# THGLab/NewtonNet

Hardware: AMD Instinct MI355X
Metric: atom-steps/sec (energy+force) on batched MD17 aspirin (higher is better)
Workload: dtype f32; 1 GPU; MD17 aspirin batched inference, 1024 conformers x 21 atoms per GPU, fp32, energy+force, neighbor list included (BASELINE.json configs[1]); 2 independent step(s) in flight per GPU; atoms_per_gpu=21504, weights=seed0, distinct_batches=4, steps_in_flight=2, parallelism=1 independent shard(s), no data-path collective

## Files before the change

newtonnet_amd/csrc/common.h:

```cpp
#pragma once
#include <hip/hip_runtime.h>
#include <stdint.h>

#include "../../include/newtonnet_hip.h"

#if (defined(EDGE_ABL_SELF) || defined(EDGE_ABL_PAIR) || defined(EDGE_ABL_TABLE) || defined(EDGE_ABL_STORE) ||              \
     defined(EDGE_ABL_NO_TABLE) || defined(EDGE_ABL_HALF_TABLE) || defined(EDGE_ABL_NOTAB) || defined(EDGE_ABL_NOMJ) || defined(MLPS_ABL_NO_H) || defined(NS_ABL_NO_Q) || defined(NS_ABL_HOT_W) || defined(MLPS_ABL_X) || defined(ABL_NO_SILU) || defined(ABL_NO_STORE) ||                  \
     (defined(LIN_ABLATE_NO_LOAD) && LIN_ABLATE_NO_LOAD) || (defined(LIN_ABLATE_NO_STORE) && LIN_ABLATE_NO_STORE) ||         \
     (defined(LIN_ABLATE_NO_MFMA) && LIN_ABLATE_NO_MFMA) || (defined(LIN_ABLATE_NO_LDS) && LIN_ABLATE_NO_LDS)) &&            \
    !defined(NNHIP_TOOLING)
#error "ablation switches produce wrong results: build through csrc/build.sh (it marks the library with -DNNHIP_TOOLING)"
#endif

#define NF NNHIP_F
#define NB NNHIP_NB
#define WAVE 64
#ifndef FT_G
#define FT_G 3072
#endif
#define FT_ROWS (FT_G + 8)
#define FT_ZERO_ROW (FT_G + 3)
#define FT_PLANE ((size_t)FT_ROWS * NNHIP_F)

typedef float f32x16 __attribute__((ext_vector_type(16)));
// ... 296 lines not shown
#define WIMG_FMT_SPLIT_F16 0
#define WIMG_FMT_BF16 1
#define WIMG_MAX_JOBS 40
struct WeightImageJobs {
  const float* src[WIMG_MAX_JOBS];
  char* dst[WIMG_MAX_JOBS];
  int fmt;
};
enum { IMG_UPDATE = 0, IMG_NODE0, IMG_NODE2, IMG_UPDATE_T, IMG_NODE0_T, IMG_NODE2_T, IMG_EQ1_0, IMG_EQ1_2, IMG_EQ2_0, IMG_EQ2_2,
       IMG_EQ1_0_T, IMG_EQ1_2_T, IMG_EQ2_0_T, IMG_EQ2_2_T, IMG_PER_LAYER };
enum { IMG_HEAD0 = 0, IMG_HEAD2, IMG_HEAD0_T, IMG_HEAD2_T, IMG_HEAD_COUNT };
struct NodeImages {
  const char *Wu, *W0, *W2;
  const char *W2T, *W0T, *WuT;
};
int launch_weight_images(const float* const* src, char* const* dst, int n, hipStream_t s, int fmt = WIMG_FMT_SPLIT_F16);
int launch_node_fwd_split(const NodeFwdArgs& a, const NodeImages& im, hipStream_t s);
int launch_node_bwd_split(const NodeBwdArgs& a, const NodeImages& im, hipStream_t s);
struct NodeTurnArgs {
  const float* f;
  const float* a_mid;
  float* a_out;
  const float *b0, *b2;
  const float *w4, *b4;
  const float *scale, *shift;
  const int64_t* z;
  float* atom_energy;
  float* g_a;
  float* gf;
  int N;
};
int launch_node_turn_split(const NodeTurnArgs& a, const NodeImages& im, hipStream_t s);
bool node_turn_enabled();
int launch_mlp_wide_split(int mode, bool accum, const MlpArgs& a, hipStream_t s);
int launch_mlp_wide_pair_split(int mode, const MlpPair& P, hipStream_t s);
int launch_lin_wide_split(const float* X, int ldx, const char* img, float* Y, int ldy, int M, bool acc, hipStream_t s);
bool split_products_enabled();

struct MsgBwdForceTail {
  const float* g_u;
  const float* geo;
  const int* rev;
  int n_edges, n_layers;
  float inv_rc;
  float* forces;
};

static inline int cdiv(long a, long b) { return (int)((a + b - 1) / b); }
```

newtonnet_amd/csrc/node128.hip:

```cpp
#include <string.h>

#include "common.h"

#ifndef NODE_WG_PER_CU
#define NODE_WG_PER_CU 2
#endif
#define NT_LD 132
#define NODE_LDS_FLOATS (32 * NT_LD)

struct Tile {
  float* xs;
  int r, h, nb;
};

__device__ __forceinline__ void load_w(float4 (&wf)[16], const Tile& t, const float* __restrict__ W) {
  const float4* wp = reinterpret_cast<const float4*>(W + (size_t)(t.nb * 32 + t.r) * NF + 4 * t.h);
#pragma unroll
  for (int k = 0; k < 16; ++k) wf[k] = wp[2 * k];
  __builtin_amdgcn_sched_barrier(0);
}

__device__ __forceinline__ f32x16 tile_gemm(const Tile& t, const float4 (&wf)[16]) {
  f32x16 acc;
#pragma unroll
// ... 57 lines not shown

__global__ void __launch_bounds__(256, NODE_WG_PER_CU) node_fwd_kernel(const NodeFwdArgs p) {
  __shared__ __attribute__((aligned(16))) float xs[NODE_LDS_FLOATS];
  Tile t;
  t.xs = xs;
  t.r = threadIdx.x & 31;
  t.h = (threadIdx.x >> 5) & 1;
  t.nb = __builtin_amdgcn_readfirstlane(threadIdx.x >> 6);
  const int row = blockIdx.x * 32 + t.r;
  const int rc = min(row, p.N - 1);
  const bool live = row < p.N;

  float4 wf[16];
  load_w(wf, t, p.Wu);
  float upd[16];
#pragma unroll
  for (int k = 0; k < 16; ++k) upd[k] = 0.f;
  float xa[16], xb[16], a[16];
  blk_load(xa, p.f, ((size_t)rc * 3 + 0) * NF, t);
#pragma unroll
  for (int c = 0; c < 3; ++c) {
    float (&cur)[16] = (c & 1) ? xb : xa;
    float (&nxt)[16] = (c & 1) ? xa : xb;
    float qv[16];
    if (c) __syncthreads();
    blk_to_tile(cur, t);
    __syncthreads();
    if (c < 2)
      blk_load(nxt, p.f, ((size_t)rc * 3 + c + 1) * NF, t);
    else
      blk_load(a, p.a_mid, (size_t)rc * NF, t);
    acc_to(qv, tile_gemm(t, wf));
    if (c == 2 && p.W0) load_w(wf, t, p.W0);
    if (live) blk_store<NODE_NT != 0>(qv, p.q, ((size_t)row * 3 + c) * NF, t);
#pragma unroll
    for (int k = 0; k < 16; ++k) upd[k] = fmaf(cur[k], qv[k], upd[k]);
  }
#pragma unroll
  for (int k = 0; k < 16; ++k) a[k] += upd[k];
  if (live) blk_store(a, p.a_out, (size_t)row * NF, t);
  if (!p.W0) return;

  __syncthreads();
  blk_to_tile(a, t);
  __syncthreads();
  float hn[16], b0v[16], b2v[16];
  blk_load(b0v, p.b0, 0, t);
  acc_to(hn, tile_gemm(t, wf));
  load_w(wf, t, p.W2);
#pragma unroll
  for (int k = 0; k < 16; ++k) hn[k] += b0v[k];
  if (live) blk_store<NODE_NT != 0>(hn, p.hn, (size_t)row * NF, t);
  NN_ACT_BLOCK(hn, 16, p.act);
  __syncthreads();
  blk_to_tile(hn, t);
  __syncthreads();
  blk_load(b2v, p.b2, 0, t);
  float m[16];
  acc_to(m, tile_gemm(t, wf));
#pragma unroll
  for (int k = 0; k < 16; ++k) m[k] += b2v[k];
  if (live) blk_store(m, p.m, (size_t)row * NF, t);
}

__global__ void __launch_bounds__(256, NODE_WG_PER_CU) node_bwd_kernel(const NodeBwdArgs p) {
  __shared__ __attribute__((aligned(16))) float xs[NODE_LDS_FLOATS];
  Tile t;
// ... 316 lines not shown
```

newtonnet_amd/csrc/node128s.hip:

```cpp
#include <stdint.h>
#include <string.h>

#include "common.h"
#include "switches.h"

typedef _Float16 h8 __attribute__((ext_vector_type(8)));
typedef _Float16 h4 __attribute__((ext_vector_type(4)));
typedef __bf16 b8 __attribute__((ext_vector_type(8)));
typedef __bf16 b4 __attribute__((ext_vector_type(4)));

#ifndef NS_WG_PER_CU
#define NS_WG_PER_CU 2
#endif
#define NS_PITCH 272
#define NS_PLANE (32 * NS_PITCH)
#define NS_LDS_BYTES (2 * NS_PLANE + 8 * 32 * 4)
#ifndef NS_MERGE3
#define NS_MERGE3 0
#endif
#define WIMG_PLANE (NF * NF * 2)

__device__ __forceinline__ void ns_pow2_scale(float m, float& S, float& inv) {
  const int e = (int)((__float_as_uint(m) >> 23) & 0xffu);
  const bool ok = e >= 40 && e < 255;
// ... 186 lines not shown
  const float4* p = reinterpret_cast<const float4*>(base + row_off + t.nb * 32 + 4 * t.h);
#pragma unroll
  for (int q = 0; q < 4; ++q) {
    const float4 x = p[2 * q];
    v[4 * q] = x.x;
    v[4 * q + 1] = x.y;
    v[4 * q + 2] = x.z;
    v[4 * q + 3] = x.w;
  }
}
__device__ __forceinline__ void sblk_store(const float (&v)[16], float* __restrict__ base, size_t row_off, const STile& t) {
  float4* p = reinterpret_cast<float4*>(base + row_off + t.nb * 32 + 4 * t.h);
#pragma unroll
  for (int q = 0; q < 4; ++q) p[2 * q] = make_float4(v[4 * q], v[4 * q + 1], v[4 * q + 2], v[4 * q + 3]);
}

#ifdef NS_CLOCK_DEBUG
#define NS_DBG_INIT() long long dbg_w[16], dbg_c[16]; int dbg_n = 0; dbg_w[0] = wall_clock64(); dbg_c[0] = clock64(); dbg_n = 1;
#define NS_DBG_STAMP() if (dbg_n < 16) { dbg_w[dbg_n] = wall_clock64(); dbg_c[dbg_n] = clock64(); ++dbg_n; }
#define NS_DBG_PRINT(tag)                                                                                      \
  NS_DBG_STAMP()                                                                                               \
  if (blockIdx.x == 0 && threadIdx.x == 0) {                                                                   \
    printf(tag " start %lld:", dbg_w[0]);                                                                      \
    for (int k_ = 1; k_ < dbg_n; ++k_)                                                                         \
      printf(" +%.2fus(%.2fGHz)", (dbg_w[k_] - dbg_w[k_ - 1]) / 100.0,                                         \
             (dbg_c[k_] - dbg_c[k_ - 1]) / ((dbg_w[k_] - dbg_w[k_ - 1]) * 10.0 + 1e-9));                        \
    printf("  end %lld\n", dbg_w[dbg_n - 1]);                                                                  \
  }
#else
#define NS_DBG_INIT()
#define NS_DBG_STAMP()
#define NS_DBG_PRINT(tag)
#endif
#define NS_TILE_SETUP()                                                      \
  __shared__ __attribute__((aligned(16))) char lds[(NS_MERGE3 ? 3 : 1) * NS_LDS_BYTES]; \
  STile t;                                                                   \
  t.img = lds;                                                               \
  t.pmax = reinterpret_cast<float*>(lds + 2 * NS_PLANE);                     \
  t.r = threadIdx.x & 31;                                                    \
  t.h = (threadIdx.x >> 5) & 1;                                              \
  t.nb = __builtin_amdgcn_readfirstlane(threadIdx.x >> 6);                   \
  const int row = blockIdx.x * 32 + t.r;                                     \
  const int rc = min(row, p.N - 1);                                          \
  const bool live = row < p.N;

__global__ void __launch_bounds__(256, NS_WG_PER_CU) node_fwd_split_kernel(const NodeFwdArgs p, const NodeImages im) {
  NS_DBG_INIT()
  NS_TILE_SETUP()
  WFrag wf;
  load_wimg(wf, t, im.Wu);
  float upd[16];
#pragma unroll
  for (int k = 0; k < 16; ++k) upd[k] = 0.f;
  float a[16];
#if NS_MERGE3
  {
    STile t1 = t, t2 = t;
    t1.img = lds + NS_LDS_BYTES;
    t1.pmax = reinterpret_cast<float*>(lds + NS_LDS_BYTES + 2 * NS_PLANE);
    t2.img = lds + 2 * NS_LDS_BYTES;
    t2.pmax = reinterpret_cast<float*>(lds + 2 * NS_LDS_BYTES + 2 * NS_PLANE);
    float x0[16], x1[16], x2[16], qv[16];
    sblk_load(x0, p.f, ((size_t)rc * 3 + 0) * NF, t);
    sblk_load(x1, p.f, ((size_t)rc * 3 + 1) * NF, t);
    sblk_load(x2, p.f, ((size_t)rc * 3 + 2) * NF, t);
    tile_publish(x0, t);
    tile_publish(x1, t1);
    tile_publish(x2, t2);
    __syncthreads();
    const float inv0 = tile_commit(x0, t), inv1 = tile_commit(x1, t1), inv2 = tile_commit(x2, t2);
    __syncthreads();
    sblk_load(a, p.a_mid, (size_t)rc * NF, t);
    tile_gemm_s(qv, t, wf, inv0);
    if (live) sblk_store(qv, p.q, ((size_t)row * 3 + 0) * NF, t);
#pragma unroll
    for (int k = 0; k < 16; ++k) upd[k] = x0[k] * qv[k];
    tile_gemm_s(qv, t1, wf, inv1);
    if (live) sblk_store(qv, p.q, ((size_t)row * 3 + 1) * NF, t);
#pragma unroll
    for (int k = 0; k < 16; ++k) upd[k] = fmaf(x1[k], qv[k], upd[k]);
    tile_gemm_s(qv, t2, wf, inv2);
    if (p.W0) load_wimg(wf, t, im.W0);
    if (live) sblk_store(qv, p.q, ((size_t)row * 3 + 2) * NF, t);
#pragma unroll
    for (int k = 0; k < 16; ++k) upd[k] = fmaf(x2[k], qv[k], upd[k]);
  }
#else
  float xa[16], xb[16];
  sblk_load(xa, p.f, ((size_t)rc * 3 + 0) * NF, t);
#pragma unroll
  for (int c = 0; c < 3; ++c) {
    float (&cur)[16] = (c & 1) ? xb : xa;
    float (&nxt)[16] = (c & 1) ? xa : xb;
    float qv[16];
    tile_publish(cur, t);
    __syncthreads();
    const float inv = tile_commit(cur, t);
    __syncthreads();
    if (c < 2)
      sblk_load(nxt, p.f, ((size_t)rc * 3 + c + 1) * NF, t);
    else
      sblk_load(a, p.a_mid, (size_t)rc * NF, t);
    NS_DBG_STAMP()
    tile_gemm_s(qv, t, wf, inv);
    NS_DBG_STAMP()
    if (c == 2 && p.W0) load_wimg(wf, t, im.W0);
#ifndef NS_ABL_NO_Q
    if (live) sblk_store(qv, p.q, ((size_t)row * 3 + c) * NF, t);
#endif
#pragma unroll
    for (int k = 0; k < 16; ++k) upd[k] = fmaf(cur[k], qv[k], upd[k]);
  }
#endif
#pragma unroll
  for (int k = 0; k < 16; ++k) a[k] += upd[k];
  if (live) sblk_store(a, p.a_out, (size_t)row * NF, t);
  if (!p.W0) return;

  tile_publish(a, t);
  __syncthreads();
  float inv = tile_commit(a, t);
  __syncthreads();
  float hn[16], b0v[16], b2v[16];
  sblk_load(b0v, p.b0, 0, t);
  NS_DBG_STAMP()
  tile_gemm_s(hn, t, wf, inv);
  NS_DBG_STAMP()
  load_wimg(wf, t, im.W2);
#pragma unroll
  for (int k = 0; k < 16; ++k) hn[k] += b0v[k];
  if (live) sblk_store(hn, p.hn, (size_t)row * NF, t);
#pragma unroll
  for (int k = 0; k < 16; ++k) hn[k] = silu_f(hn[k]);
  tile_publish(hn, t);
  __syncthreads();
  inv = tile_commit(hn, t);
  __syncthreads();
  sblk_load(b2v, p.b2, 0, t);
  float m[16];
  NS_DBG_STAMP()
  tile_gemm_s(m, t, wf, inv);
  NS_DBG_STAMP()
#pragma unroll
  for (int k = 0; k < 16; ++k) m[k] += b2v[k];
  if (live) sblk_store(m, p.m, (size_t)row * NF, t);
  NS_DBG_PRINT("node_fwd")
}

#ifndef NS_WG_PER_CU_BWD
#define NS_WG_PER_CU_BWD NS_WG_PER_CU
#endif
__global__ void __launch_bounds__(256, NS_WG_PER_CU_BWD) node_bwd_split_kernel(const NodeBwdArgs p, const NodeImages im) {
  NS_TILE_SETUP()
  float ga[16];
  WFrag wf;
  if (p.W2T) {
    load_wimg(wf, t, im.W2T);
    float x[16], hpre[16], g[16];
    sblk_load(x, p.g_top, (size_t)rc * NF, t);
    sblk_load(hpre, p.h_top, (size_t)rc * NF, t);
    tile_publish(x, t);
    __syncthreads();
    float inv = tile_commit(x, t);
    __syncthreads();
    tile_gemm_s(g, t, wf, inv);
    load_wimg(wf, t, im.W0T);
    if (p.T && live) sblk_store(g, p.T, (size_t)row * NF, t);
#pragma unroll
    for (int k = 0; k < 16; ++k) g[k] *= dsilu_f(hpre[k]);
    tile_publish(g, t);
    __syncthreads();
    inv = tile_commit(g, t);
    __syncthreads();
    tile_gemm_s(ga, t, wf, inv);
    if (p.WuT) load_wimg(wf, t, im.WuT);
    if (p.acc_ga) {
      float old[16];
      sblk_load(old, p.g_a_in ? p.g_a_in : p.g_a, (size_t)rc * NF, t);
#pragma unroll
      for (int k = 0; k < 16; ++k) ga[k] += old[k];
    }
    if (live) sblk_store(ga, p.g_a, (size_t)row * NF, t);
  } else {
    sblk_load(ga, p.g_a, (size_t)rc * NF, t);
    if (p.WuT) load_wimg(wf, t, im.WuT);
  }
// ... 10 lines not shown
    sblk_load(x0, p.f, ((size_t)rc * 3 + 0) * NF, t);
    sblk_load(x1, p.f, ((size_t)rc * 3 + 1) * NF, t);
    sblk_load(x2, p.f, ((size_t)rc * 3 + 2) * NF, t);
#pragma unroll
    for (int k = 0; k < 16; ++k) {
      x0[k] *= ga[k];
      x1[k] *= ga[k];
      x2[k] *= ga[k];
    }
    tile_publish(x0, t);
    tile_publish(x1, t1);
    tile_publish(x2, t2);
    __syncthreads();
    const float inv0 = tile_commit(x0, t), inv1 = tile_commit(x1, t1), inv2 = tile_commit(x2, t2);
    __syncthreads();
#pragma unroll
    for (int c = 0; c < 3; ++c) {
      float out[16], qv[16], gin[16];
      sblk_load(qv, p.q, ((size_t)rc * 3 + c) * NF, t);
      if (p.G_f) sblk_load(gin, p.G_f, ((size_t)rc * 3 + c) * NF, t);
      tile_gemm_s(out, c == 0 ? t : (c == 1 ? t1 : t2), wf, c == 0 ? inv0 : (c == 1 ? inv1 : inv2));
#pragma unroll
      for (int k = 0; k < 16; ++k) out[k] = fmaf(ga[k], qv[k], out[k]);
      if (p.G_f) {
#pragma unroll
        for (int k = 0; k < 16; ++k) out[k] += gin[k];
      }
      if (live) sblk_store(out, p.gf, ((size_t)row * 3 + c) * NF, t);
    }
  }
#else
  float fa[16], fb[16];
  sblk_load(fa, p.f, ((size_t)rc * 3 + 0) * NF, t);
#pragma unroll
  for (int c = 0; c < 3; ++c) {
    float (&cur)[16] = (c & 1) ? fb : fa;
    float (&nxt)[16] = (c & 1) ? fa : fb;
    float out[16], qv[16], gin[16];
#pragma unroll
    for (int k = 0; k < 16; ++k) cur[k] *= ga[k];
    tile_publish(cur, t);
    __syncthreads();
    const float inv = tile_commit(cur, t);
    __syncthreads();
    if (c < 2) sblk_load(nxt, p.f, ((size_t)rc * 3 + c + 1) * NF, t);
#ifdef NS_ABL_NO_Q
#pragma unroll
    for (int k = 0; k < 16; ++k) qv[k] = cur[k];
#else
    sblk_load(qv, p.q, ((size_t)rc * 3 + c) * NF, t);
#endif
    if (p.G_f) sblk_load(gin, p.G_f, ((size_t)rc * 3 + c) * NF, t);
    tile_gemm_s(out, t, wf, inv);
#pragma unroll
    for (int k = 0; k < 16; ++k) out[k] = fmaf(ga[k], qv[k], out[k]);
    if (p.G_f) {
#pragma unroll
      for (int k = 0; k < 16; ++k) out[k] += gin[k];
    }
    if (live) sblk_store(out, p.gf, ((size_t)row * 3 + c) * NF, t);
  }
#endif
}

#define NT_PITCH 132
static_assert(32 * NT_PITCH * 4 <= 2 * NS_PLANE, "the fp32 e2 tile must fit in the f16 planes of the LDS tile");
__global__ void __launch_bounds__(256, NS_WG_PER_CU_BWD) node_turn_split_kernel(const NodeTurnArgs p, const NodeImages im) {
  NS_TILE_SETUP()
  WFrag wf;
  load_wimg(wf, t, im.Wu);
  float fk[3][16], qk[3][16], a[16];
  {
    float upd[16];
#pragma unroll
    for (int k = 0; k < 16; ++k) upd[k] = 0.f;
    sblk_load(fk[0], p.f, ((size_t)rc * 3 + 0) * NF, t);
#pragma unroll
    for (int c = 0; c < 3; ++c) {
      tile_publish(fk[c], t);
      __syncthreads();
      const float inv = tile_commit(fk[c], t);
      __syncthreads();
      if (c < 2)
        sblk_load(fk[c + 1], p.f, ((size_t)rc * 3 + c + 1) * NF, t);
      else
        sblk_load(a, p.a_mid, (size_t)rc * NF, t);
      tile_gemm_s(qk[c], t, wf, inv);
      if (c == 2) load_wimg(wf, t, im.W0);
#pragma unroll
      for (int k = 0; k < 16; ++k) upd[k] = fmaf(fk[c][k], qk[c][k], upd[k]);
    }
#pragma unroll
    for (int k = 0; k < 16; ++k) a[k] += upd[k];
// ... 216 lines not shown
      for (int k = 0; k < 16; ++k) out[k] += gin[k];
    }
    if (live) sblk_store(out, p.dgf, ooff, t);
  }
}

int launch_node_tan_fwd_split(const NodeTanFwdArgs& a, const NodeImages& im, hipStream_t s) {
  if (a.N <= 0) return 0;
  ScopedTimer t0(TC_LIN, s);
  node_tan_fwd_split_kernel<<<cdiv(a.N, 32), 256, 0, s>>>(a, im);
  LAUNCH_CHECK();
  return 0;
}
int launch_node_tan_bwd_split(const NodeTanBwdArgs& a, const NodeImages& im, hipStream_t s) {
  if (a.N <= 0) return 0;
  ScopedTimer t0(TC_LIN, s);
  node_tan_bwd_split_kernel<<<cdiv(a.N, 32), 256, 0, s>>>(a, im);
  LAUNCH_CHECK();
  return 0;
}

int launch_node_fwd_split(const NodeFwdArgs& a, const NodeImages& im, hipStream_t s) {
  if (a.N <= 0) return 0;
  ScopedTimer t0(TC_LIN, s);
  ScopedTimer t1(TC_LIN1, s);
  node_fwd_split_kernel<<<cdiv(a.N, 32), 256, 0, s>>>(a, im);
  LAUNCH_CHECK();
  return 0;
}
int launch_node_bwd_split(const NodeBwdArgs& a, const NodeImages& im, hipStream_t s) {
  if (a.N <= 0) return 0;
  ScopedTimer t0(TC_LIN, s);
  ScopedTimer t1(TC_LIN1, s);
  node_bwd_split_kernel<<<cdiv(a.N, 32), 256, 0, s>>>(a, im);
  LAUNCH_CHECK();
  return 0;
}

bool node_turn_enabled() { return switches().node_turn != 0; }
int launch_node_turn_split(const NodeTurnArgs& a, const NodeImages& im, hipStream_t s) {
  if (a.N <= 0) return 0;
  ScopedTimer t0(TC_LIN, s);
  ScopedTimer t1(TC_LIN1, s);
  node_turn_split_kernel<<<cdiv(a.N, 32), 256, 0, s>>>(a, im);
  LAUNCH_CHECK();
  return 0;
}

template <int MODE>
__device__ __forceinline__ void mlp_wide_split_body(const MlpArgs& p, const bool accum, STile& t) {
  const int M = mlp_rows(p);
  if ((int)blockIdx.x * 32 >= M) return;
  const int row = blockIdx.x * 32 + t.r;
  const int rc = min(row, M - 1);
  const bool live = row < M;

  const bool bf = wimg_is_bf16(p.W1_img);
  WFrag wf;
  load_wimg(wf, t, p.W1_img);
  float x[16], hv[16], hin[16];
  sblk_load(x, p.X, (size_t)rc * p.ldx, t);
  if (MODE != MODE_FWD) sblk_load(hin, p.H, (size_t)rc * p.ldh, t);
  float inv = 1.0f;
  if (bf) {
    __syncthreads();
    tile_commit_bf(x, t);
    __syncthreads();
    tile_gemm_bf(hv, t, wf);
  } else {
    tile_publish(x, t);
// ... 177 lines not shown
```

newtonnet_amd/csrc/pipeline.hip:

```cpp
#include <stdarg.h>
#include <stdio.h>
#include <string.h>

#include <atomic>
#include <mutex>
#include <algorithm>
#include <vector>

#include "common.h"
#include "switches.h"

int launch_filter_tables(const float* const* edge_w, float* const* tables, int n_layers, const float* freq, int nb,
                         int envelope, hipStream_t s);
int launch_msg_fwd(const float* m, const int* xg, const float* table, const int* row_ptr, const int* col,
                   const int* pid, const float* a_in, float* msg, float* a_mid, int n_atoms, hipStream_t s);
int launch_force_fwd(bool has_f, const float* phi1, const float* phi2, const float* geo, const int* row_ptr,
                     const int* col, const int* pid, const float* f_in, float* f_out, int n_atoms, const int* xg, hipStream_t s,
                     const int* pair_ptr = nullptr, const int* mol_ptr = nullptr, int n_mol = 0);
int launch_force_bwd(bool has_f, const float* gf, const float* phi1, const float* phi2, const float* geo,
                     const int* row_ptr, const int* col, const int* pid, const float* f_in, float* g_h12, float* g_u,
                     float* g_fin, int n_atoms, const int* xg, hipStream_t s, const int* pair_ptr = nullptr, const int* rev = nullptr);
int launch_msg_bwd(const float* g_msg, const float* g_a, const float* m, const int* xg, const float* table,
                   const int* row_ptr, const int* col, const int* pid, float* g_m, float* g_x, int n_atoms, bool need_gm,
                   hipStream_t s, const int* pair_ptr = nullptr, const int* mol_ptr = nullptr, int n_mol = 0,
// ... 36 lines not shown
extern "C" int nnhip_mlp_forms(void);
extern "C" int nnhip_graph_small_max_atoms(void);
static bool graph_mol_on() { return switches().graph_mol != 0; }
extern "C" int nnhip_config(char* buf, size_t n) {
  if (!buf || n < 64) {
    nnhip_set_error("nnhip_config: buffer of at least 64 bytes");
    return NNHIP_E_INVALID;
  }
  std::vector<const char*> names(std::begin(kSwitchNames), std::end(kSwitchNames));
  names.insert(names.end(), std::begin(kPythonSwitchNames), std::end(kPythonSwitchNames));
  std::sort(names.begin(), names.end(), [](const char* a, const char* b) { return strcmp(a, b) < 0; });
  int small_atoms, mol_min, wpr[4], mol_forms;
  edge_config(&small_atoms, &mol_min, wpr, &mol_forms);
  const int forms = nnhip_mlp_forms();
  size_t o = 0;
  auto put = [&](const char* fmt, auto... a) {
    if (o < n) {
      const int k = snprintf(buf + o, n - o, fmt, a...);
      o += k > 0 ? (size_t)k : 0;
    }
  };
  put("{\"version\": %d, \"tooling_build\": %d, \"split_f16_products\": %d, ", nnhip_version(), nnhip_build_flags(), forms & 1);
  put("\"neighbor_list\": {\"single_launch_max_atoms\": %d, \"per_molecule_kernels\": %d, \"cell_list\": \"one periodic molecule (host choice)\"}, ",
      nnhip_graph_small_max_atoms(), graph_mol_on() ? 1 : 0);
  put("\"edge_rows\": {\"waves_per_row\": {\"msg_fwd\": %d, \"force_fwd\": %d, \"force_bwd\": %d, \"msg_bwd\": %d}, \"four_waves_per_row_up_to_atoms\": %d}, ",
      wpr[0], wpr[1], wpr[2], wpr[3], small_atoms);
  put("\"molecule_forms\": {\"max_atoms\": %d, \"edge_kernels_from_molecules\": %d, \"force_fwd\": %d, \"msg_bwd\": %d, \"force_direct\": %d, \"head_out\": %d, "
      "\"msg_bwd_with_forces\": %d}, ",
      NNHIP_MOL_STAGE_MAX, mol_min, mol_forms & 1, (mol_forms >> 1) & 1, (mol_forms >> 2) & 1, (mol_forms >> 3) & 1, (mol_forms >> 4) & 1);
  put("\"edge_mlp\": {\"row_local_up_to_tiles\": %d, \"one_pass_adjoint\": %d, \"one_pass_forward\": %d, \"one_pass_single_adjoint\": %d, "
      "\"one_pass_single_forward\": %d}, ",
      mlp_wide_max_tiles_silu(), (forms >> 1) & 1, (forms >> 2) & 1, (forms >> 3) & 1, (forms >> 4) & 1);
  put("\"node_turn_fused\": %d, ", ((forms & 1) && node_turn_enabled()) ? 1 : 0);
  put("\"radial_table_intervals\": %d, \"env\": {", FT_G);
  bool first = true;
  for (const char* nm : names) {
    const char* v = switch_text(nm);
    if (!v) continue;
    char clean[25];
    int k = 0;
    for (; k < 24 && v[k]; ++k) {
      const char ch = v[k];
      const bool ok = (ch >= '0' && ch <= '9') || (ch >= 'a' && ch <= 'z') || (ch >= 'A' && ch <= 'Z') || ch == '_' || ch == '.' ||
                      ch == ',' || ch == '+' || ch == '-';
      clean[k] = ok ? ch : '?';
    }
    clean[k] = 0;
    put("%s\"%s\": \"%s\"", first ? "" : ", ", nm, clean);
    first = false;
  }
  put("%s", "}}");
  if (o >= n) {
    nnhip_set_error("nnhip_config: buffer of %zu bytes is too small", n);
    return NNHIP_E_INVALID;
  }
  return NNHIP_OK;
}

struct TimerRec {
  int cls;
  hipEvent_t e0, e1;
};
static std::atomic<bool> g_timers_on{false};
static std::atomic<uint32_t> g_timer_mask{0xffffffffu};
static std::mutex g_timer_mu;
static std::vector<TimerRec> g_pending;
// ... 482 lines not shown
  }
  const int P_ = E / 2;
  const size_t h2_off = (size_t)((P_ + 31) / 32 * 32) * NF;
  WsInternal w;
  make_layout(N, E, B, L, w);
  if (workspace_bytes < w.pub.total || (!workspace && w.pub.total)) {
    nnhip_set_error("nnhip_energy_forces: workspace %zu < required %zu bytes", workspace_bytes, w.pub.total);
    return NNHIP_E_WORKSPACE;
  }
  if (((uintptr_t)workspace & 255) != 0) {
    nnhip_set_error("nnhip_energy_forces: workspace must be 256-byte aligned");
    return NNHIP_E_INVALID;
  }
  if (N == 0) {
    if (B > 0) HIP_TRY(hipMemsetAsync(energy, 0, sizeof(float) * B, s));
    return NNHIP_OK;
  }
  char* ws = (char*)workspace;
  auto P = [&](size_t off) { return (float*)(ws + off); };
  const bool want_forces = forces != nullptr;

  PrepLayout pq;
  make_prep_layout(L, pq);
  char* pbase = prepared ? (char*)prepared : ws + w.prep;
  auto Q = [&](size_t off) { return (float*)(pbase + off); };
  if (!prepared) TRY(run_prepare(model, pq, pbase, s));
  const bool split_nodes = split_products_enabled() && act == NNHIP_ACT_SILU;
  if (!embedded) TRY(launch_embed(z, model->node_embedding, Q(pq.m_tab), N, P(w.pub.a0), P(w.pub.m[0]), s));
  const float* a_in = P(w.pub.a0);
  const float* f_in = nullptr;
  auto A_OUT = [&](int l) { return (l == L - 1 && atom_node_out) ? atom_node_out : P(w.pub.a_out[l]); };
  auto F_OUT = [&](int l) { return (l == L - 1 && force_node_out) ? force_node_out : P(w.pub.f_out[l]); };
  const bool node_turn = split_nodes && want_forces && !model->layer[L - 1].ln_w && node_turn_enabled();
  for (int l = 0; l < L; ++l) {
    const nnhip_layer_params& lp = model->layer[l];
    const bool has_f = l > 0;
    {
      TRY(launch_msg_fwd(P(w.pub.m[l]), xg, Q(pq.ftab[l]), row_ptr, col, pid, a_in, P(w.pub.msg[l]), P(w.pub.a_mid[l]), N, s));
      if (E > 0) {
        float* h12 = P(w.pub.h12[l]);
        MlpArgs m1 = {P(w.pub.msg[l]), lp.eq1_0_w, lp.eq1_2_w, h12, P(w.pub.phi1[l]), P_, NF, NF, NF};
        MlpArgs m2 = {P(w.pub.msg[l]), lp.eq2_0_w, lp.eq2_2_w, h12 + h2_off, P(w.pub.phi2[l]), P_, NF, NF, NF};
        m1.h_frag = m2.h_frag = 1;
        m1.act = m2.act = act;
        m1.M_dev = m2.M_dev = n_pairs_dev;
        if (split_nodes) {
          m1.W1_img = pbase + pq.img[l][IMG_EQ1_0];
          m1.W2_img = pbase + pq.img[l][IMG_EQ1_2];
          m2.W1_img = pbase + pq.img[l][IMG_EQ2_0];
          m2.W2_img = pbase + pq.img[l][IMG_EQ2_2];
        }
        if (has_f)
          TRY(launch_mlp_pair(MODE_FWD, m1, false, m2, false, s));
        else
          TRY(launch_mlp(MODE_FWD, false, m1, s));
      }
      TRY(launch_force_fwd(has_f, P(w.pub.phi1[l]), P(w.pub.phi2[l]), geo, row_ptr, col, pid, f_in, F_OUT(l), N, mask_xg, s, pair_ptr,
                           mol_kernels ? mol_ptr : nullptr, B));
    }
    if (!(node_turn && l == L - 1)) {
      NodeFwdArgs na;
      memset(&na, 0, sizeof(na));
      na.f = F_OUT(l);
      na.a_mid = P(w.pub.a_mid[l]);
      na.Wu = lp.update_w;
      na.q = P(w.pub.q[l]);
      na.a_out = A_OUT(l);
      if (l + 1 < L && !lp.ln_w) {
        const nnhip_layer_params& nx = model->layer[l + 1];
        na.W0 = nx.node0_w;
        na.b0 = nx.node0_b;
        na.W2 = nx.node2_w;
        na.b2 = nx.node2_b;
        na.hn = P(w.pub.hn[l + 1]);
        na.m = P(w.pub.m[l + 1]);
      } else if (l + 1 == L && !lp.ln_w) {
        na.W0 = model->head0_w;
        na.b0 = model->head0_b;
        na.W2 = model->head2_w;
        na.b2 = model->head2_b;
        na.hn = P(w.pub.e1);
        na.m = P(w.pub.e2);
      }
      na.N = N;
      na.act = act;
      if (split_nodes) {
        NodeImages im;
        memset(&im, 0, sizeof(im));
        im.Wu = pbase + pq.img[l][IMG_UPDATE];
        if (na.W0) {
          im.W0 = l + 1 < L ? pbase + pq.img[l + 1][IMG_NODE0] : pbase + pq.img_head[IMG_HEAD0];
          im.W2 = l + 1 < L ? pbase + pq.img[l + 1][IMG_NODE2] : pbase + pq.img_head[IMG_HEAD2];
        }
        TRY(launch_node_fwd_split(na, im, s));
      } else {
        TRY(launch_node_fwd(na, s));
      }
    }
    if (lp.ln_w) {
// ... 27 lines not shown
    nt.atom_energy = atom_energy;
    nt.g_a = P(w.pub.g_a);
    nt.gf = P(w.gf_mid);
    nt.N = N;
    NodeImages im;
    memset(&im, 0, sizeof(im));
    im.Wu = pbase + pq.img[L - 1][IMG_UPDATE];
    im.W0 = pbase + pq.img_head[IMG_HEAD0];
    im.W2 = pbase + pq.img_head[IMG_HEAD2];
    im.W2T = pbase + pq.img_head[IMG_HEAD2_T];
    im.W0T = pbase + pq.img_head[IMG_HEAD0_T];
    im.WuT = pbase + pq.img[L - 1][IMG_UPDATE_T];
    TRY(launch_node_turn_split(nt, im, s));
    TRY(launch_mol_energy(atom_energy, mol_ptr, N, B, energy, s, mol_kernels));
  } else {
    TRY(launch_head_out(P(w.pub.e2), model->head4_w, model->head4_b, model->scale, model->shift, z, mol_ptr, N, B,
                        act, atom_energy, want_forces ? P(w.g_e) : nullptr, energy, s, mol_kernels));
  }
  if (!want_forces) return NNHIP_OK;

  auto node_bwd = [&](const NodeBwdArgs& a, const NodeImages& im) {
    return split_nodes ? launch_node_bwd_split(a, im, s) : launch_node_bwd(a, s);
  };
  if (!node_turn) {
    NodeBwdArgs nb;
    memset(&nb, 0, sizeof(nb));
    nb.g_top = P(w.g_e);
    nb.h_top = P(w.pub.e1);
    nb.W2T = Q(pq.headT[1]);
    nb.W0T = Q(pq.headT[0]);
    nb.g_a = P(w.pub.g_a);
    nb.acc_ga = 0;
    nb.f = F_OUT(L - 1);
    nb.q = P(w.pub.q[L - 1]);
    nb.G_f = nullptr;
    nb.WuT = Q(pq.wT[L - 1][6]);
    nb.gf = P(w.gf_mid);
    nb.N = N;
    nb.act = act;
    NodeImages bim;
    memset(&bim, 0, sizeof(bim));
    bim.W2T = pbase + pq.img_head[IMG_HEAD2_T];
    bim.W0T = pbase + pq.img_head[IMG_HEAD0_T];
    bim.WuT = pbase + pq.img[L - 1][IMG_UPDATE_T];
    const nnhip_layer_params& top = model->layer[L - 1];
    if (top.ln_w) {
      NodeBwdArgs head = nb;
      head.WuT = nullptr;
      TRY(node_bwd(head, bim));
      TRY(launch_layer_norm_bwd(P(w.pub.g_a), top.ln_w, P(w.xhat[L - 1]), P(w.rstd[L - 1]), N, s));
      nb.W2T = nullptr;
    }
    TRY(node_bwd(nb, bim));
  }
  float* g_fbuf[2] = {P(w.pub.g_f), P(w.g_f2)};
  int pp = 0;
  MsgBwdForceTail ftail = {P(w.pub.g_u), geo, rev, E, L, 1.0f / model->cutoff, forces};
  const bool ftail_ok = mol_kernels && !virial && B > 0 && (long)N <= (long)B * NNHIP_MOL_STAGE_MAX;
  bool forces_done = false;
  for (int l = L - 1; l >= 0; --l) {
    const nnhip_layer_params& lp = model->layer[l];
    (void)lp;
    const bool has_f = l > 0;
    const float* f_prev = has_f ? F_OUT(l - 1) : nullptr;
    float* g_fin = g_fbuf[pp];
    {
      TRY(launch_force_bwd(has_f, P(w.gf_mid), P(w.pub.phi1[l]), P(w.pub.phi2[l]), geo, row_ptr, col, pid, f_prev,
                           P(w.g_h12), P(w.pub.g_u) + (size_t)l * E * 4, g_fin, N, mask_xg, s, pair_ptr, rev));
      if (E > 0) {
        float* gp = P(w.g_h12);
        float* h12 = P(w.pub.h12[l]);
        MlpArgs m1 = {gp, Q(pq.wT[l][3]), Q(pq.wT[l][2]), h12, P(w.g_msg), P_, 2 * NF, NF, NF};
        MlpArgs m2 = {gp + NF, Q(pq.wT[l][5]), Q(pq.wT[l][4]), h12 + h2_off, P(w.g_msg), P_, 2 * NF, NF, NF};
        m1.h_frag = m2.h_frag = 1;
        m1.act = m2.act = act;
        m1.M_dev = m2.M_dev = n_pairs_dev;
        if (split_nodes) {
          m1.W1_img = pbase + pq.img[l][IMG_EQ1_2_T];
          m1.W2_img = pbase + pq.img[l][IMG_EQ1_0_T];
          m2.W1_img = pbase + pq.img[l][IMG_EQ2_2_T];
          m2.W2_img = pbase + pq.img[l][IMG_EQ2_0_T];
        }
        if (has_f)
          TRY(launch_mlp_pair(MODE_BWD, m1, false, m2, true, s));
        else
          TRY(launch_mlp(MODE_BWD, false, m1, s));
      }
      TRY(launch_msg_bwd(P(w.g_msg), P(w.pub.g_a), P(w.pub.m[l]), xg, Q(pq.ftab[l]), row_ptr, col, pid, P(w.g_m),
                         P(w.pub.g_x) + (size_t)l * E, N, l > 0, s, pair_ptr, mol_kernels ? mol_ptr : nullptr, B,
                         (l == 0 && ftail_ok) ? &ftail : nullptr, &forces_done));
    }
    if (l > 0) {
      NodeBwdArgs nb;
      memset(&nb, 0, sizeof(nb));
      nb.g_top = P(w.g_m);
      nb.h_top = P(w.pub.hn[l]);
      nb.W2T = Q(pq.wT[l][1]);
      nb.W0T = Q(pq.wT[l][0]);
      nb.g_a = P(w.pub.g_a);
      nb.acc_ga = 1;
      nb.f = F_OUT(l - 1);
      nb.q = P(w.pub.q[l - 1]);
      nb.G_f = g_fin;
      nb.WuT = Q(pq.wT[l - 1][6]);
      nb.gf = P(w.gf_mid);
      nb.N = N;
      nb.act = act;
      NodeImages bim;
      memset(&bim, 0, sizeof(bim));
      bim.W2T = pbase + pq.img[l][IMG_NODE2_T];
      bim.W0T = pbase + pq.img[l][IMG_NODE0_T];
      bim.WuT = pbase + pq.img[l - 1][IMG_UPDATE_T];
      const nnhip_layer_params& below = model->layer[l - 1];
      if (below.ln_w) {
        NodeBwdArgs mlp = nb;
        mlp.WuT = nullptr;
        TRY(node_bwd(mlp, bim));
        TRY(launch_layer_norm_bwd(P(w.pub.g_a), below.ln_w, P(w.xhat[l - 1]), P(w.rstd[l - 1]), N, s));
        nb.W2T = nullptr;
      }
      TRY(node_bwd(nb, bim));
    }
    pp ^= 1;
  }
  if (!forces_done)
    TRY(launch_geometry_bwd(P(w.pub.g_x), P(w.pub.g_u), geo, disp, pos, cell, row_ptr, col, rev, mol_ptr, N, E, B, L,
                            model->cutoff, P(w.g_d), forces, virial, s, mol_kernels));
  return NNHIP_OK;
}

extern "C" int nnhip_energy_forces(const nnhip_model* model, const int64_t* z, const float* pos, const float* cell,
                                   const int32_t* mol_ptr, const int32_t* row_ptr, const int32_t* col,
                                   const int32_t* rev, const int32_t* pid, const float* geo, const int32_t* xg,
                                   const float* disp, int32_t N, int32_t E, int32_t B, void* workspace,
                                   size_t workspace_bytes, float* energy, float* forces, float* virial,
                                   float* atom_energy_out, float* atom_node_out, float* force_node_out,
                                   const void* prepared, void* stream_) {
  return energy_forces_impl(model, z, pos, cell, mol_ptr, row_ptr, col, rev, pid, geo, xg, disp, N, E, B, workspace, workspace_bytes,
                            energy, forces, virial, atom_energy_out, atom_node_out, force_node_out, prepared, nullptr, nullptr,
                            stream_);
}
extern "C" int nnhip_energy_forces_pp(const nnhip_model* model, const int64_t* z, const float* pos, const float* cell,
                                      const int32_t* mol_ptr, const int32_t* row_ptr, const int32_t* col,
                                      const int32_t* rev, const int32_t* pid, const float* geo, const int32_t* xg,
                                      const float* disp, int32_t N, int32_t E, int32_t B, void* workspace,
// ... 207 lines not shown
```

newtonnet_amd/csrc/switches.h:

```cpp
#pragma once
#include <stdlib.h>

#ifndef EDGE_SMALL_ATOMS
#define EDGE_SMALL_ATOMS 2048
#endif

#define NNHIP_SWITCH_TABLE(X)                                                                                                      \
  X(long, lnum, edge_lds, "NNHIP_EDGE_LDS", 0)                         \
  X(int, num, edge_small_atoms, "NNHIP_EDGE_SMALL_ATOMS", EDGE_SMALL_ATOMS)  \
  X(int, num, edge_wpr, "NNHIP_EDGE_WPR", 0)                           \
  X(int, flag, force_bwd_owner_gu, "NNHIP_FORCE_BWD_OWNER_GU", 1)      \
  X(int, flag, force_direct_mol, "NNHIP_FORCE_DIRECT_MOL", 1)          \
  X(int, flag, force_fwd_mol, "NNHIP_FORCE_FWD_MOL", 1)                \
  X(int, flag, graph_mol, "NNHIP_GRAPH_MOL", 1)                        \
  X(int, num, graph_small_atoms, "NNHIP_GRAPH_SMALL_ATOMS", 128)       \
  X(int, flag, head_out_mol, "NNHIP_HEAD_OUT_MOL", 1)                  \
  X(int, num, lin_blocks, "NNHIP_LIN_BLOCKS", 512)                     \
  X(int, num, mlp_regw, "NNHIP_MLP_REGW", 1)                           \
  X(int, num, mlp_regw_single, "NNHIP_MLP_REGW_SINGLE", 1)             \
  X(int, flag, mlp_regw_train, "NNHIP_MLP_REGW_TRAIN", 1)              \
  X(int, flag, mlp_split, "NNHIP_MLP_SPLIT", 1)                        \
  X(int, num, mlp_wide_tiles, "NNHIP_MLP_WIDE_TILES", -1)              \
  X(int, num, mol_kernels_min, "NNHIP_MOL_KERNELS_MIN", 640)           \
  X(int, flag, msg_bwd_force, "NNHIP_MSG_BWD_FORCE", 1)                \
  X(int, flag, msg_bwd_mol, "NNHIP_MSG_BWD_MOL", 1)                    \
  X(int, flag, node_turn, "NNHIP_NODE_TURN", 1)

struct Switches {
#define X(type, kind, field, name, dflt) type field;
  NNHIP_SWITCH_TABLE(X)
#undef X
};

inline const char* const kSwitchNames[] = {
#define X(type, kind, field, name, dflt) name,
    NNHIP_SWITCH_TABLE(X)
#undef X
};
inline const char* const kPythonSwitchNames[] = {"NNHIP_TRAIN_BF16", "NNHIP_WGRAD_FORM", "NNHIP_WGRAD_RPC"};

inline const char* switch_text(const char* name) { return getenv(name); }
inline int switch_flag(const char* v, int) { return (v && atoi(v) == 0) ? 0 : 1; }
inline int switch_num(const char* v, int dflt) { return v ? atoi(v) : dflt; }
inline long switch_lnum(const char* v, long dflt) { return v ? atol(v) : dflt; }

inline const Switches& switches() {
  static const Switches sw = [] {
    Switches s;
#define X(type, kind, field, name, dflt) s.field = switch_##kind(switch_text(name), dflt);
    NNHIP_SWITCH_TABLE(X)
#undef X
    if (s.edge_wpr != 1 && s.edge_wpr != 2 && s.edge_wpr != 4) s.edge_wpr = 0;
    if (s.mlp_wide_tiles < 0) s.mlp_wide_tiles = -1;
    return s;
  }();
  return sw;
}
```

Baseline: 15.79 million atom-steps/s.

## Recompute q in node backward instead of storing it in forward

The forward node kernels skip writing the per-atom q tensor (3×N×F) when no buffer is passed. The backward split kernel gains a template variant that rebuilds q by running an extra tile GEMM of f against the update-weight image, using a second LDS tile. This trades a large global write plus read of q for extra matrix math and double the LDS per workgroup in the backward kernel, which may lower occupancy. A switch controls it and it is on by default for layers without layer norm.

Result: faster. 16.16 million atom-steps/s, median of 6 (+2.4%).

```diff
diff --git a/newtonnet_amd/csrc/common.h b/newtonnet_amd/csrc/common.h
--- a/newtonnet_amd/csrc/common.h
+++ b/newtonnet_amd/csrc/common.h
@@ -352,6 +352,7 @@
 };
 int launch_node_turn_split(const NodeTurnArgs& a, const NodeImages& im, hipStream_t s);
 bool node_turn_enabled();
+bool node_bwd_q_enabled();
 int launch_mlp_wide_split(int mode, bool accum, const MlpArgs& a, hipStream_t s);
 int launch_mlp_wide_pair_split(int mode, const MlpPair& P, hipStream_t s);
 int launch_lin_wide_split(const float* X, int ldx, const char* img, float* Y, int ldy, int M, bool acc, hipStream_t s);
diff --git a/newtonnet_amd/csrc/node128.hip b/newtonnet_amd/csrc/node128.hip
--- a/newtonnet_amd/csrc/node128.hip
+++ b/newtonnet_amd/csrc/node128.hip
@@ -113,7 +113,7 @@
       blk_load(a, p.a_mid, (size_t)rc * NF, t);
     acc_to(qv, tile_gemm(t, wf));
     if (c == 2 && p.W0) load_w(wf, t, p.W0);
-    if (live) blk_store<NODE_NT != 0>(qv, p.q, ((size_t)row * 3 + c) * NF, t);
+    if (p.q && live) blk_store<NODE_NT != 0>(qv, p.q, ((size_t)row * 3 + c) * NF, t);
 #pragma unroll
     for (int k = 0; k < 16; ++k) upd[k] = fmaf(cur[k], qv[k], upd[k]);
   }
diff --git a/newtonnet_amd/csrc/node128s.hip b/newtonnet_amd/csrc/node128s.hip
--- a/newtonnet_amd/csrc/node128s.hip
+++ b/newtonnet_amd/csrc/node128s.hip
@@ -242,8 +242,8 @@
 #define NS_DBG_STAMP()
 #define NS_DBG_PRINT(tag)
 #endif
-#define NS_TILE_SETUP()                                                      \
-  __shared__ __attribute__((aligned(16))) char lds[(NS_MERGE3 ? 3 : 1) * NS_LDS_BYTES]; \
+#define NS_TILE_SETUP_N(NTILES)                                              \
+  __shared__ __attribute__((aligned(16))) char lds[(NTILES) * NS_LDS_BYTES]; \
   STile t;                                                                   \
   t.img = lds;                                                               \
   t.pmax = reinterpret_cast<float*>(lds + 2 * NS_PLANE);                     \
@@ -253,6 +253,7 @@
   const int row = blockIdx.x * 32 + t.r;                                     \
   const int rc = min(row, p.N - 1);                                          \
   const bool live = row < p.N;
+#define NS_TILE_SETUP() NS_TILE_SETUP_N(NS_MERGE3 ? 3 : 1)
 
 __global__ void __launch_bounds__(256, NS_WG_PER_CU) node_fwd_split_kernel(const NodeFwdArgs p, const NodeImages im) {
   NS_DBG_INIT()
@@ -282,16 +283,16 @@
     __syncthreads();
     sblk_load(a, p.a_mid, (size_t)rc * NF, t);
     tile_gemm_s(qv, t, wf, inv0);
-    if (live) sblk_store(qv, p.q, ((size_t)row * 3 + 0) * NF, t);
+    if (p.q && live) sblk_store(qv, p.q, ((size_t)row * 3 + 0) * NF, t);
 #pragma unroll
     for (int k = 0; k < 16; ++k) upd[k] = x0[k] * qv[k];
     tile_gemm_s(qv, t1, wf, inv1);
-    if (live) sblk_store(qv, p.q, ((size_t)row * 3 + 1) * NF, t);
+    if (p.q && live) sblk_store(qv, p.q, ((size_t)row * 3 + 1) * NF, t);
 #pragma unroll
     for (int k = 0; k < 16; ++k) upd[k] = fmaf(x1[k], qv[k], upd[k]);
     tile_gemm_s(qv, t2, wf, inv2);
     if (p.W0) load_wimg(wf, t, im.W0);
-    if (live) sblk_store(qv, p.q, ((size_t)row * 3 + 2) * NF, t);
+    if (p.q && live) sblk_store(qv, p.q, ((size_t)row * 3 + 2) * NF, t);
 #pragma unroll
     for (int k = 0; k < 16; ++k) upd[k] = fmaf(x2[k], qv[k], upd[k]);
   }
@@ -316,7 +317,7 @@
     NS_DBG_STAMP()
     if (c == 2 && p.W0) load_wimg(wf, t, im.W0);
 #ifndef NS_ABL_NO_Q
-    if (live) sblk_store(qv, p.q, ((size_t)row * 3 + c) * NF, t);
+    if (p.q && live) sblk_store(qv, p.q, ((size_t)row * 3 + c) * NF, t);
 #endif
 #pragma unroll
     for (int k = 0; k < 16; ++k) upd[k] = fmaf(cur[k], qv[k], upd[k]);
@@ -360,8 +361,9 @@
 #ifndef NS_WG_PER_CU_BWD
 #define NS_WG_PER_CU_BWD NS_WG_PER_CU
 #endif
+template <bool RQ>
 __global__ void __launch_bounds__(256, NS_WG_PER_CU_BWD) node_bwd_split_kernel(const NodeBwdArgs p, const NodeImages im) {
-  NS_TILE_SETUP()
+  NS_TILE_SETUP_N(NS_MERGE3 ? 3 : (RQ ? 2 : 1))
   float ga[16];
   WFrag wf;
   if (p.W2T) {
@@ -438,33 +440,66 @@
 #else
   float fa[16], fb[16];
   sblk_load(fa, p.f, ((size_t)rc * 3 + 0) * NF, t);
-#pragma unroll
-  for (int c = 0; c < 3; ++c) {
-    float (&cur)[16] = (c & 1) ? fb : fa;
-    float (&nxt)[16] = (c & 1) ? fa : fb;
-    float out[16], qv[16], gin[16];
-#pragma unroll
-    for (int k = 0; k < 16; ++k) cur[k] *= ga[k];
-    tile_publish(cur, t);
-    __syncthreads();
-    const float inv = tile_commit(cur, t);
-    __syncthreads();
-    if (c < 2) sblk_load(nxt, p.f, ((size_t)rc * 3 + c + 1) * NF, t);
+  if constexpr (RQ) {
+    WFrag wq;
+    load_wimg(wq, t, im.Wu);
+    STile tg = t;
+    tg.img = lds + NS_LDS_BYTES;
+    tg.pmax = reinterpret_cast<float*>(lds + NS_LDS_BYTES + 2 * NS_PLANE);
+#pragma unroll
+    for (int c = 0; c < 3; ++c) {
+      float (&cur)[16] = (c & 1) ? fb : fa;
+      float (&nxt)[16] = (c & 1) ? fa : fb;
+      float out[16], qv[16], gin[16], gq[16];
+#pragma unroll
+      for (int k = 0; k < 16; ++k) gq[k] = cur[k] * ga[k];
+      tile_publish(cur, t);
+      tile_publish(gq, tg);
+      __syncthreads();
+      const float invf = tile_commit(cur, t);
+      const float invg = tile_commit(gq, tg);
+      __syncthreads();
+      if (c < 2) sblk_load(nxt, p.f, ((size_t)rc * 3 + c + 1) * NF, t);
+      if (p.G_f) sblk_load(gin, p.G_f, ((size_t)rc * 3 + c) * NF, t);
+      tile_gemm_s(qv, t, wq, invf);
+      tile_gemm_s(out, tg, wf, invg);
+#pragma unroll
+      for (int k = 0; k < 16; ++k) out[k] = fmaf(ga[k], qv[k], out[k]);
+      if (p.G_f) {
+#pragma unroll
+        for (int k = 0; k < 16; ++k) out[k] += gin[k];
+      }
+      if (live) sblk_store(out, p.gf, ((size_t)row * 3 + c) * NF, t);
+    }
+  } else {
+#pragma unroll
+    for (int c = 0; c < 3; ++c) {
+      float (&cur)[16] = (c & 1) ? fb : fa;
+      float (&nxt)[16] = (c & 1) ? fa : fb;
+      float out[16], qv[16], gin[16];
+#pragma unroll
+      for (int k = 0; k < 16; ++k) cur[k] *= ga[k];
+      tile_publish(cur, t);
+      __syncthreads();
+      const float inv = tile_commit(cur, t);
+      __syncthreads();
+      if (c < 2) sblk_load(nxt, p.f, ((size_t)rc * 3 + c + 1) * NF, t);
 #ifdef NS_ABL_NO_Q
 #pragma unroll
-    for (int k = 0; k < 16; ++k) qv[k] = cur[k];
+      for (int k = 0; k < 16; ++k) qv[k] = cur[k];
 #else
-    sblk_load(qv, p.q, ((size_t)rc * 3 + c) * NF, t);
+      sblk_load(qv, p.q, ((size_t)rc * 3 + c) * NF, t);
 #endif
-    if (p.G_f) sblk_load(gin, p.G_f, ((size_t)rc * 3 + c) * NF, t);
-    tile_gemm_s(out, t, wf, inv);
-#pragma unroll
-    for (int k = 0; k < 16; ++k) out[k] = fmaf(ga[k], qv[k], out[k]);
-    if (p.G_f) {
-#pragma unroll
-      for (int k = 0; k < 16; ++k) out[k] += gin[k];
-    }
-    if (live) sblk_store(out, p.gf, ((size_t)row * 3 + c) * NF, t);
+      if (p.G_f) sblk_load(gin, p.G_f, ((size_t)rc * 3 + c) * NF, t);
+      tile_gemm_s(out, t, wf, inv);
+#pragma unroll
+      for (int k = 0; k < 16; ++k) out[k] = fmaf(ga[k], qv[k], out[k]);
+      if (p.G_f) {
+#pragma unroll
+        for (int k = 0; k < 16; ++k) out[k] += gin[k];
+      }
+      if (live) sblk_store(out, p.gf, ((size_t)row * 3 + c) * NF, t);
+    }
   }
 #endif
 }
@@ -747,10 +782,19 @@
   if (a.N <= 0) return 0;
   ScopedTimer t0(TC_LIN, s);
   ScopedTimer t1(TC_LIN1, s);
-  node_bwd_split_kernel<<<cdiv(a.N, 32), 256, 0, s>>>(a, im);
+  if (a.WuT && !a.q) {
+    if (!im.Wu || NS_MERGE3) {
+      nnhip_set_error("node_bwd: no q and no image of the update weights to form it from");
+      return NNHIP_E_INVALID;
+    }
+    node_bwd_split_kernel<true><<<cdiv(a.N, 32), 256, 0, s>>>(a, im);
+  } else {
+    node_bwd_split_kernel<false><<<cdiv(a.N, 32), 256, 0, s>>>(a, im);
+  }
   LAUNCH_CHECK();
   return 0;
 }
+bool node_bwd_q_enabled() { return !NS_MERGE3 && switches().node_bwd_q != 0; }
 
 bool node_turn_enabled() { return switches().node_turn != 0; }
 int launch_node_turn_split(const NodeTurnArgs& a, const NodeImages& im, hipStream_t s) {
diff --git a/newtonnet_amd/csrc/pipeline.hip b/newtonnet_amd/csrc/pipeline.hip
--- a/newtonnet_amd/csrc/pipeline.hip
+++ b/newtonnet_amd/csrc/pipeline.hip
@@ -92,6 +92,7 @@
       "\"one_pass_single_forward\": %d}, ",
       mlp_wide_max_tiles_silu(), (forms >> 1) & 1, (forms >> 2) & 1, (forms >> 3) & 1, (forms >> 4) & 1);
   put("\"node_turn_fused\": %d, ", ((forms & 1) && node_turn_enabled()) ? 1 : 0);
+  put("\"node_bwd_recomputes_q\": %d, ", ((forms & 1) && node_bwd_q_enabled()) ? 1 : 0);
   put("\"radial_table_intervals\": %d, \"env\": {", FT_G);
   bool first = true;
   for (const char* nm : names) {
@@ -640,6 +641,8 @@
   auto A_OUT = [&](int l) { return (l == L - 1 && atom_node_out) ? atom_node_out : P(w.pub.a_out[l]); };
   auto F_OUT = [&](int l) { return (l == L - 1 && force_node_out) ? force_node_out : P(w.pub.f_out[l]); };
   const bool node_turn = split_nodes && want_forces && !model->layer[L - 1].ln_w && node_turn_enabled();
+  const bool recompute_q = split_nodes && want_forces && node_bwd_q_enabled();
+  auto q_stored = [&](int l) { return want_forces && !(recompute_q && !model->layer[l].ln_w); };
   for (int l = 0; l < L; ++l) {
     const nnhip_layer_params& lp = model->layer[l];
     const bool has_f = l > 0;
@@ -672,7 +675,7 @@
       na.f = F_OUT(l);
       na.a_mid = P(w.pub.a_mid[l]);
       na.Wu = lp.update_w;
-      na.q = P(w.pub.q[l]);
+      na.q = q_stored(l) ? P(w.pub.q[l]) : nullptr;
       na.a_out = A_OUT(l);
       if (l + 1 < L && !lp.ln_w) {
         const nnhip_layer_params& nx = model->layer[l + 1];
@@ -766,7 +769,7 @@
     nb.g_a = P(w.pub.g_a);
     nb.acc_ga = 0;
     nb.f = F_OUT(L - 1);
-    nb.q = P(w.pub.q[L - 1]);
+    nb.q = q_stored(L - 1) ? P(w.pub.q[L - 1]) : nullptr;
     nb.G_f = nullptr;
     nb.WuT = Q(pq.wT[L - 1][6]);
     nb.gf = P(w.gf_mid);
@@ -777,6 +780,7 @@
     bim.W2T = pbase + pq.img_head[IMG_HEAD2_T];
     bim.W0T = pbase + pq.img_head[IMG_HEAD0_T];
     bim.WuT = pbase + pq.img[L - 1][IMG_UPDATE_T];
+    bim.Wu = pbase + pq.img[L - 1][IMG_UPDATE];
     const nnhip_layer_params& top = model->layer[L - 1];
     if (top.ln_w) {
       NodeBwdArgs head = nb;
@@ -834,7 +838,7 @@
       nb.g_a = P(w.pub.g_a);
       nb.acc_ga = 1;
       nb.f = F_OUT(l - 1);
-      nb.q = P(w.pub.q[l - 1]);
+      nb.q = q_stored(l - 1) ? P(w.pub.q[l - 1]) : nullptr;
       nb.G_f = g_fin;
       nb.WuT = Q(pq.wT[l - 1][6]);
       nb.gf = P(w.gf_mid);
@@ -845,6 +849,7 @@
       bim.W2T = pbase + pq.img[l][IMG_NODE2_T];
       bim.W0T = pbase + pq.img[l][IMG_NODE0_T];
       bim.WuT = pbase + pq.img[l - 1][IMG_UPDATE_T];
+      bim.Wu = pbase + pq.img[l - 1][IMG_UPDATE];
       const nnhip_layer_params& below = model->layer[l - 1];
       if (below.ln_w) {
         NodeBwdArgs mlp = nb;
diff --git a/newtonnet_amd/csrc/switches.h b/newtonnet_amd/csrc/switches.h
--- a/newtonnet_amd/csrc/switches.h
+++ b/newtonnet_amd/csrc/switches.h
@@ -24,6 +24,7 @@
   X(int, num, mol_kernels_min, "NNHIP_MOL_KERNELS_MIN", 640)           \
   X(int, flag, msg_bwd_force, "NNHIP_MSG_BWD_FORCE", 1)                \
   X(int, flag, msg_bwd_mol, "NNHIP_MSG_BWD_MOL", 1)                    \
+  X(int, flag, node_bwd_q, "NNHIP_NODE_BWD_Q", 1)                      \
   X(int, flag, node_turn, "NNHIP_NODE_TURN", 1)
 
 struct Switches {
```
